# hiroharu-kato/neural_renderer

Hardware: AMD Instinct MI355X
Metric: rasterize fwd+bwd Mpixels/sec @256x256 batch=64 (higher is better)
Workload: dtype f32

## Files before the change

neural_renderer_amd/csrc/nr_backward_pixel_map.hip:

```cpp
#include "nr_device.h"
#include "nr_band_lines.h"
#include "nr_k6_tune.h"

#include <atomic>
#include <mutex>
#include <type_traits>

using namespace nr;

namespace {

constexpr int GRP = 10;
constexpr int NGRP = 6;

struct __attribute__((aligned(16))) LineRec {
    int in_rng;
    int out_rng;
    int base;
    int flags;
    float cross, c0, c1, pad;
    float in_c[4];
    float out_c[4];
};

// ... 101 lines not shown
        const int nl = lane_on ? min(max(n_lines - batch0, 0), GRP) : 0;
        int l = -1, ph = 0, d1 = 0, d1_end = -1, base = 0, cur_flags = 0;
        float cross = 0, c0 = 0, c1 = 0, ref_a = 0, ref_r = 0, ref_g = 0, ref_b = 0;
        while (__ballot(l < nl) != 0ull) {
            if (d1 > d1_end && l < nl) {
                if (ph == 0 && (cur_flags & 2)) ph = 1; else { ph = 0; ++l; }
                if (l < nl) {
                    const LineRec *r = &recs[g][l];
                    const int4 h = *reinterpret_cast<const int4 *>(r);
                    const float4 q = *reinterpret_cast<const float4 *>(&r->cross);
                    const float4 col = *reinterpret_cast<const float4 *>(ph == 0 ? r->out_c : r->in_c);
                    const int rng = ph == 0 ? h.x : h.y;
                    d1 = (rng & 0xffff) + sub;
                    d1_end = rng >> 16;
                    base = h.z;
                    cur_flags = h.w;
                    cross = q.x; c0 = q.y; c1 = q.z;
                    ref_a = col.x; ref_r = col.y; ref_g = col.z; ref_b = col.w;
                }
            }
            if (l < nl && d1 <= d1_end) {
                const int idx = base + d1 * sd1;
                bool skip = (ph == 0) && (fi_map[idx] != fn);
                float diff = 0.0f;
                if (!skip) {
                    if (ALPHA) diff += (alpha_map[idx] - ref_a) * g_alpha[idx];
                    if (RGB) {
                        const float *pp = rgb_map + 3 * (size_t)idx;
                        const float *gg = g_rgb + 3 * (size_t)idx;
                        diff += (pp[0] - ref_r) * gg[0];
                        diff += (pp[1] - ref_g) * gg[1];
                        diff += (pp[2] - ref_b) * gg[2];
                    }
                }
                if (!skip && !(diff <= 0.0f)) {
                    const float t = (float)d1 - cross;
                    if (cur_flags & 4) {
                        const float ct = c0 * t;
                        float dist = (float)(s_pow2 ? (double)ct * two_over_s : (double)ct * 2.0 / s_d);
                        dist = (0.0f < dist) ? (float)((double)dist + eps) : (float)((double)dist - eps);
                        G0 -= (double)(diff / dist);
                    }
                    if (cur_flags & 8) {
                        const float ct = c1 * t;
                        float dist = (float)(s_pow2 ? (double)ct * two_over_s : (double)ct * 2.0 / s_d);
                        dist = (0.0f < dist) ? (float)((double)dist + eps) : (float)((double)dist - eps);
                        G1 -= (double)(diff / dist);
                    }
                }
                d1 += GRP;
            }
        }
        __syncthreads();
    }

#pragma unroll
    for (int o = 8; o > 0; o >>= 1) {
        const double t0 = __shfl_down(G0, o, WAVE), t1 = __shfl_down(G1, o, WAVE);
        if (sub + o < GRP) { G0 += t0; G1 += t1; }
    }
    const int partner = (2 * ((edge + 2) % 3) + axis) * GRP;
    const double G1p = __shfl(G1, partner, WAVE);
    if (lane_on && sub == 0) {
        out[3 * edge + (1 - axis)] = (float)(G0 + G1p);
        if (axis == 0) out[3 * edge + 2] = 0.0f;
    }
}


constexpr int BAND_WIN = 256;
constexpr int FSEG = 15;
enum { K6_FAST = 0, K6_EXACT_POW2 = 1, K6_EXACT = 2 };

__global__ __launch_bounds__(256) void k_mark_visible(const int32_t *__restrict__ fi_map,
                                                      unsigned char *__restrict__ flags, int F, int SS, size_t P)
{
    const size_t i = (size_t)blockIdx.x * blockDim.x + threadIdx.x;
    if (i >= P) return;
    const int fi = fi_map[i];
    if (fi >= 0) flags[(i / SS) * F + fi] = 1;
}

__device__ __forceinline__ void emit_visible(int b, int fn, int pos, int F, int S, const float *__restrict__ faces,
                                             int *__restrict__ vis_list, unsigned *__restrict__ rng,
                                             double *__restrict__ scratch, int *band_count, int n_bands, int W,
                                             int *line_diff = nullptr)
{
    vis_list[(size_t)b * F + pos] = fn;
    const float *f = faces + ((size_t)b * F + fn) * 9;
    const float fs = (float)S;
    float px[3], py[3];
#pragma unroll
    for (int k = 0; k < 3; k++) { px[k] = to_pixel(f[3 * k], fs); py[k] = to_pixel(f[3 * k + 1], fs); }
    unsigned *r0 = rng + (((size_t)b * 2 + 0) * F + pos) * 3, *r1 = rng + (((size_t)b * 2 + 1) * F + pos) * 3;
#pragma unroll
    for (int e = 0; e < 3; e++) {
        const unsigned ra = edge_range(px[e], px[(e + 1) % 3], S), rb = edge_range(py[e], py[(e + 1) % 3], S);
        r0[e] = ra;
        r1[e] = rb;
#pragma unroll
        for (int axis = 0; axis < 2; axis++) {
            const unsigned r = axis ? rb : ra;
            const int lo = (int)(r & 0xffffu), hi = (int)(r >> 16);
            if (line_diff) {
                if (lo <= hi) {
                    atomicAdd(line_diff + axis * (S + 1) + lo, 1);
                    atomicAdd(line_diff + axis * (S + 1) + hi + 1, -1);
                }
                continue;
            }
            for (int band = lo / W; band * W <= hi; ++band)
                atomicAdd(band_count + axis * n_bands + band, min(hi, band * W + W - 1) - max(lo, band * W) + 1);
        }
    }
    double2 *z = reinterpret_cast<double2 *>(scratch + ((size_t)b * F + pos) * 6);
    z[0] = z[1] = z[2] = make_double2(0.0, 0.0);
}

__device__ __forceinline__ void zero_face(float *__restrict__ o)
{
#pragma unroll
    for (int k = 0; k < 9; k++) o[k] = 0.0f;
}

constexpr int VIS_CHUNK = 1024;
constexpr int SMALL_CHUNKS = 16;

__global__ __launch_bounds__(VIS_CHUNK) void k_compact_par(const unsigned char *__restrict__ flags,
                                                           int *__restrict__ vis_list, int *__restrict__ vis_count,
                                                           int *__restrict__ slot_of, int F, int n_chunks,
                                                           const float *__restrict__ faces, unsigned *__restrict__ rng,
                                                           double *__restrict__ scratch, int S,
                                                           int *__restrict__ chunk_band, int n_bands, int W,
                                                           int *__restrict__ band_cursor, float *__restrict__ zero_faces,
                                                           int zero_listed, int use_diff)
{
    extern __shared__ int s_band[];
    __shared__ int s_wcnt[VIS_CHUNK / 64];
    __shared__ int s_part[VIS_CHUNK / 64];
    const int b = blockIdx.y, chunk = blockIdx.x, tid = threadIdx.x, lane = tid & 63, wave = tid >> 6;
    for (int i = tid; i < 2 * n_bands; i += VIS_CHUNK) s_band[i] = 0;
    int *s_diff = use_diff ? s_band + 2 * n_bands : nullptr;
    if (use_diff)
        for (int i = tid; i < 2 * (S + 1); i += VIS_CHUNK) s_diff[i] = 0;
    int part = 0;
    for (int c = 0; c < chunk; ++c) part += __popcll(__ballot(flags[(size_t)b * F + c * VIS_CHUNK + tid] != 0));
    const int fn = chunk * VIS_CHUNK + tid;
    const bool v = fn < F && flags[(size_t)b * F + fn] != 0;
    const unsigned long long m = __ballot(v);
    if (lane == 0) { s_part[wave] = part; s_wcnt[wave] = __popcll(m); }
    __syncthreads();
    int off = 0, own = 0;
    for (int w = 0; w < VIS_CHUNK / 64; ++w) {
        off += s_part[w];
        if (w < wave) off += s_wcnt[w];
        own += s_wcnt[w];
    }
    if (fn < F) {
        const int before = off + __popcll(m & ((1ull << lane) - 1ull));
        slot_of[(size_t)b * F + fn] = v ? before : -1;
        if (v) emit_visible(b, fn, before, F, S, faces, vis_list, rng, scratch, s_band, n_bands, W, s_diff);
        if (zero_faces && (!v || zero_listed)) zero_face(zero_faces + ((size_t)b * F + fn) * 9);
    }
    __syncthreads();
    if (use_diff) {
        const int n2 = 2 * (S + 1), per = (n2 + VIS_CHUNK - 1) / VIS_CHUNK, i0 = tid * per, i1 = min(n2, i0 + per);
        int local = 0;
        for (int i = i0; i < i1; ++i) local += s_diff[i];
        int inc = local;
#pragma unroll
        for (int o = 1; o < 64; o <<= 1) {
            const int t = __shfl_up(inc, o, WAVE);
            if (lane >= o) inc += t;
        }
        __syncthreads();
        if (lane == 63) s_wcnt[wave] = inc;
        __syncthreads();
        int run = inc - local;
        for (int w = 0; w < wave; ++w) run += s_wcnt[w];
        for (int i = i0; i < i1; ++i) {
            run += s_diff[i];
            s_diff[i] = run;
        }
        __syncthreads();
        for (int i = tid; i < 2 * n_bands; i += VIS_CHUNK) {
            const int axis = i >= n_bands, band = i - axis * n_bands;
            int c = 0;
            for (int l = band * W; l < min(S, band * W + W); ++l) c += s_diff[axis * (S + 1) + l];
            s_band[i] = c;
        }
        __syncthreads();
    }
    int *row = chunk_band + ((size_t)b * n_chunks + chunk) * 2 * n_bands;
    for (int i = tid; i < 2 * n_bands; i += VIS_CHUNK) row[i] = s_band[i];
    if (chunk == 0)
        for (int i = tid; i < 2 * n_bands; i += VIS_CHUNK) band_cursor[(size_t)b * 2 * n_bands + i] = 0;
    if (chunk == n_chunks - 1 && tid == 0) {
        int base = 0;
        for (int w = 0; w < VIS_CHUNK / 64; ++w) base += s_part[w];
        vis_count[b] = base + own;
    }
}

__global__ __launch_bounds__(VIS_CHUNK) void k_list_visible(const unsigned char *__restrict__ flags,
                                                            int *__restrict__ vis_list, int *__restrict__ vis_count, int F,
                                                            int n_chunks)
{
    __shared__ int s_wcnt[VIS_CHUNK / 64];
    __shared__ int s_part[VIS_CHUNK / 64];
    const int b = blockIdx.y, chunk = blockIdx.x, tid = threadIdx.x, lane = tid & 63, wave = tid >> 6;
    int part = 0;
    for (int c = 0; c < chunk; ++c) part += __popcll(__ballot(flags[(size_t)b * F + c * VIS_CHUNK + tid] != 0));
    const int fn = chunk * VIS_CHUNK + tid;
    const bool v = fn < F && flags[(size_t)b * F + fn] != 0;
    const unsigned long long m = __ballot(v);
    if (lane == 0) { s_part[wave] = part; s_wcnt[wave] = __popcll(m); }
    __syncthreads();
    int off = 0, own = 0;
    for (int w = 0; w < VIS_CHUNK / 64; ++w) {
        off += s_part[w];
        if (w < wave) off += s_wcnt[w];
        own += s_wcnt[w];
    }
    if (v) vis_list[(size_t)b * F + off + __popcll(m & ((1ull << lane) - 1ull))] = fn;
    if (chunk == n_chunks - 1 && tid == 0) {
        int base = 0;
        for (int w = 0; w < VIS_CHUNK / 64; ++w) base += s_part[w];
        vis_count[b] = base + own;
    }
}

__global__ __launch_bounds__(VIS_CHUNK) void k_count_visible(const unsigned char *__restrict__ flags,
                                                             int *__restrict__ chunk_count, int F, int n_chunks,
                                                             int *__restrict__ band_lines, int n_bands)
{
    __shared__ int s_wcnt[VIS_CHUNK / 64];
    const int b = blockIdx.y, chunk = blockIdx.x, tid = threadIdx.x, lane = tid & 63, wave = tid >> 6;
    for (int i = chunk * VIS_CHUNK + tid; i < 2 * n_bands; i += n_chunks * VIS_CHUNK) band_lines[(size_t)b * 2 * n_bands + i] = 0;
    const int fn = chunk * VIS_CHUNK + tid;
    const bool v = fn < F && flags[(size_t)b * F + fn] != 0;
    const unsigned long long m = __ballot(v);
    if (lane == 0) s_wcnt[wave] = __popcll(m);
    __syncthreads();
    if (tid == 0) {
        int tot = 0;
        for (int w = 0; w < VIS_CHUNK / 64; ++w) tot += s_wcnt[w];
        chunk_count[(size_t)b * n_chunks + chunk] = tot;
    }
}

__global__ __launch_bounds__(VIS_CHUNK) void k_compact_visible(const unsigned char *__restrict__ flags,
                                                               const int *__restrict__ chunk_count,
                                                               int *__restrict__ vis_list, int *__restrict__ vis_count,
                                                               int *__restrict__ slot_of, int F, int n_chunks,
                                                               const float *__restrict__ faces,
                                                               unsigned *__restrict__ rng, double *__restrict__ scratch,
                                                               int S, int *__restrict__ band_lines, int n_bands, int W,
                                                               int lds_counters, float *__restrict__ zero_faces,
                                                               int zero_listed)
{
    extern __shared__ int s_band[];
    __shared__ int s_wcnt[VIS_CHUNK / 64];
    __shared__ int s_part[VIS_CHUNK / 64];
    const int b = blockIdx.y, chunk = blockIdx.x, tid = threadIdx.x, lane = tid & 63, wave = tid >> 6;
    if (lds_counters)
        for (int i = tid; i < 2 * n_bands; i += VIS_CHUNK) s_band[i] = 0;
    int part = 0;
    for (int c = tid; c < chunk; c += VIS_CHUNK) part += chunk_count[(size_t)b * n_chunks + c];
#pragma unroll
    for (int o = 32; o > 0; o >>= 1) part += __shfl_xor(part, o, WAVE);
    const int fn = chunk * VIS_CHUNK + tid;
    const bool v = fn < F && flags[(size_t)b * F + fn] != 0;
    const unsigned long long m = __ballot(v);
    if (lane == 0) { s_part[wave] = part; s_wcnt[wave] = __popcll(m); }
    __syncthreads();
    int off = 0, own = 0;
    for (int w = 0; w < VIS_CHUNK / 64; ++w) {
        off += s_part[w];
        if (w < wave) off += s_wcnt[w];
        own += s_wcnt[w];
    }
    if (fn < F) {
        const int before = off + __popcll(m & ((1ull << lane) - 1ull));
        slot_of[(size_t)b * F + fn] = v ? before : -1;
        if (zero_faces && (!v || zero_listed)) zero_face(zero_faces + ((size_t)b * F + fn) * 9);
        if (v)
            emit_visible(b, fn, before, F, S, faces, vis_list, rng, scratch,
                         lds_counters ? s_band : band_lines + (size_t)b * 2 * n_bands, n_bands, W);
    }
    if (lds_counters) {
        __syncthreads();
        for (int i = tid; i < 2 * n_bands; i += VIS_CHUNK) {
            const int c = s_band[i];
            if (c) atomicAdd(band_lines + (size_t)b * 2 * n_bands + i, c);
        }
    }
    if (chunk == n_chunks - 1 && tid == 0) {
        int base = 0;
        for (int w = 0; w < VIS_CHUNK / 64; ++w) base += s_part[w];
        vis_count[b] = base + own;
    }
}

template <int NT>
__device__ __forceinline__ int block_excl_scan(int v, int *s_tmp, int *total)
{
    const int tid = threadIdx.x, lane = tid & 63, wave = tid >> 6;
    int inc = v;
#pragma unroll
    for (int o = 1; o < 64; o <<= 1) {
        const int t = __shfl_up(inc, o, WAVE);
        if (lane >= o) inc += t;
    }
    if (lane == 63) s_tmp[wave] = inc;
    __syncthreads();
    int woff = 0, tot = 0;
    for (int w = 0; w < NT / 64; ++w) {
        const int c = s_tmp[w];
        if (w < wave) woff += c;
        tot += c;
    }
    __syncthreads();
    *total = tot;
    return woff + inc - v;
}

__device__ __forceinline__ double signed_eps(float dist, unsigned eps_hi, unsigned eps_lo)
{
    return __hiloint2double((int)((0.0f < dist) ? eps_hi : (eps_hi ^ 0x80000000u)), (int)eps_lo);
}

__global__ __launch_bounds__(256) void k_line_setup(LineSetupArgs a) { line_setup_body(a, (int)blockIdx.x, (int)blockIdx.y); }

__device__ __forceinline__ void band_prefix(const int *cnt, int n2, int *__restrict__ start_out, int *__restrict__ cursor_out,
                                            int *__restrict__ ok_out, size_t cap)
{
    if (threadIdx.x >= 64) return;
    const int lane = threadIdx.x, per = (n2 + 63) / 64;
    int local = 0;
    for (int i = lane * per; i < min(n2, (lane + 1) * per); ++i) local += cnt[i];
    int inc = local;
#pragma unroll
    for (int o = 1; o < 64; o <<= 1) {
        const int t = __shfl_up(inc, o, WAVE);
        if (lane >= o) inc += t;
    }
    int run = inc - local;
    for (int i = lane * per; i < min(n2, (lane + 1) * per); ++i) {
        start_out[i] = run;
        cursor_out[i] = 0;
        run += cnt[i];
    }
    const int total = __shfl(inc, 63, WAVE);
    if (lane == 0) *ok_out = ((size_t)total <= cap) ? 1 : 0;
}

__global__ __launch_bounds__(256) void k_band_scan(const int *__restrict__ band_lines, int *__restrict__ band_start,
                                                   int *__restrict__ band_cursor, int *__restrict__ lines_ok, int n_bands,
                                                   size_t cap, int force_scan)
{
    const size_t o = (size_t)blockIdx.x * 2 * n_bands;
    band_prefix(band_lines + o, 2 * n_bands, band_start + o, band_cursor + o, lines_ok + blockIdx.x, force_scan ? 0 : cap);
}

__global__ __launch_bounds__(256) void k_band_total(const int *__restrict__ chunk_band, int n_sum, int *__restrict__ band_lines,
                                                    int *__restrict__ band_start, int *__restrict__ lines_ok, int n_bands)
{
    const int b = blockIdx.x, n2 = 2 * n_bands;
    const int *rows = chunk_band + (size_t)b * n_sum * n2;
    for (int i = threadIdx.x; i < n2; i += blockDim.x) {
        int t = 0;
        for (int c = 0; c < n_sum; ++c) t += rows[(size_t)c * n2 + i];
        band_lines[(size_t)b * n2 + i] = t;
        band_start[(size_t)b * n2 + i] = 0;
    }
    if (threadIdx.x == 0) lines_ok[b] = 0;
}

struct FastPx {
    int *fi;
    float *g;
    float *c;
    float *bg;
    unsigned *cov;
    int CW;
    int *span;
};

template <bool RGB, bool ALPHA, int NT>
__device__ __forceinline__ void fast_stage(const FastPx &px, const int32_t *__restrict__ fi_map,
                                           const float *__restrict__ rgb_map, const float *__restrict__ alpha_map,
                                           const float *__restrict__ g_rgb, const float *__restrict__ g_alpha, size_t img,
                                           int axis, int band_lo, int nld, int S, int SP)
{
    const int tid = threadIdx.x;
    auto put = [&](int ld, int d1, int fi, float al, float ga, float r, float g, float bl, float gr, float gg, float gb) {
        const int l = ld * SP + d1;
        px.fi[l] = fi;
        if (RGB) {
            *reinterpret_cast<float4 *>(px.g + 4 * (size_t)l) = make_float4(ga, gr, gg, gb);
            *reinterpret_cast<float4 *>(px.c + 4 * (size_t)l) = make_float4(al, r, g, bl);
            if (px.bg && fi < 0) *reinterpret_cast<float4 *>(px.bg) = make_float4(al, r, g, bl);
        } else {
            px.g[l] = ga;
            px.c[l] = al;
            if (px.bg && fi < 0) px.bg[0] = al;
        }
        if (px.cov && fi >= 0) atomicOr(px.cov + ld * px.CW + (d1 >> 5), 1u << (d1 & 31));
    };
    auto put_quad = [&](size_t g, int ld0, int d10, int ld_step, int d1_step) {
        const int4 vf = *reinterpret_cast<const int4 *>(fi_map + g);
        float4 va = make_float4(0, 0, 0, 0), vg = va;
        if (ALPHA) {
            va = *reinterpret_cast<const float4 *>(alpha_map + g);
            vg = *reinterpret_cast<const float4 *>(g_alpha + g);
// ... 1106 lines not shown
                            used(gD);
                            __builtin_amdgcn_sched_barrier(0);
                            gp += 4 * (SEG * NC * 4);
                            pp += 4 * SEG;
                            pf += (float)(4 * SEG);
                        }
                        if (const int rem = steps2 - s) {
                            if (rem == 3) load(2, gC, pC);
                            visit(gA, pA, pf, a0, a1);
                            used(gA);
                            if (rem >= 2) {
                                visit(gB, pB, pf + (float)SEG, b0, b1);
                                used(gB);
                            }
                            if (rem == 3) {
                                visit(gC, pC, pf + (float)(2 * SEG), a0, a1);
                                used(gC);
                            }
                        }
                    }
                    A0 = __builtin_amdgcn_mfma_f64_4x4x4f64((double)a0, 1.0, 0.0, 0, 0, 0);
                    A1 = __builtin_amdgcn_mfma_f64_4x4x4f64((double)a1, 1.0, 0.0, 0, 0, 0);
                    A0 = __builtin_amdgcn_mfma_f64_4x4x4f64((double)b0, 1.0, A0, 0, 0, 0);
                    A1 = __builtin_amdgcn_mfma_f64_4x4x4f64((double)b1, 1.0, A1, 0, 0, 0);
                    A0 = __builtin_amdgcn_mfma_f64_4x4x4f64(A0, 1.0, 0.0, 0, 0, 0);
                    A1 = __builtin_amdgcn_mfma_f64_4x4x4f64(A1, 1.0, 0.0, 0, 0, 0);
                }
                if (act && lane == (row << 2)) acc[src] = make_double2(A0, A1);
            }
            wave_lds_handover();
            if (lane < nw) {
                double2 a = make_double2(0.0, 0.0);
                if (has_b && ((pos >> 2) & (team - 1)) == member) a = acc[lane];
                a.x += (double)f0;
                a.y += (double)f1;
                const bool tneg = !dpos;
                const bool neg0 = EXACT || (((__float_as_uint(qq.y) >> 31) != 0) != tneg);
                const bool neg1 = EXACT || (((__float_as_uint(qq.z) >> 31) != 0) != tneg);
                const double t0 = (flags & 2) ? in0 + (neg0 ? a.x : -a.x) : 0.0;
                const double t1 = (flags & 4) ? in1 + (neg1 ? a.y : -a.y) : 0.0;
                const int tgt = hh.w, lpos = tgt & 0x0fffffff;
                double *dst = scratch + ((size_t)b * F + lpos) * 6 + (1 - axis);
                if (t0 != 0.0) atomicAdd(dst + 2 * ((tgt >> 28) & 3), t0);
                if (t1 != 0.0) atomicAdd(dst + 2 * ((tgt >> 30) & 3), t1);
            }
            wave_lds_handover();
        }
    }
}

__global__ __launch_bounds__(256) void k_bpm_finalize(const double *__restrict__ scratch, const int *__restrict__ slot_of,
                                                      float *__restrict__ grad_faces, int F, int n_faces_total, int add)
{
    const int i = blockIdx.x * blockDim.x + threadIdx.x;
    if (i >= n_faces_total) return;
    const int pos = slot_of[i];
    float *o = grad_faces + (size_t)i * 9;
    if (add) {
        if (pos < 0) return;
        const double *src = scratch + ((size_t)(i / F) * F + pos) * 6;
#pragma unroll
        for (int v = 0; v < 3; v++) {
            o[3 * v + 0] = (float)src[2 * v + 0] + o[3 * v + 0];
            o[3 * v + 1] = (float)src[2 * v + 1] + o[3 * v + 1];
        }
        return;
    }
    double a[6] = {0.0, 0.0, 0.0, 0.0, 0.0, 0.0};
    if (pos >= 0) {
        const double *src = scratch + ((size_t)(i / F) * F + pos) * 6;
#pragma unroll
        for (int k = 0; k < 6; k++) a[k] = src[k];
    }
#pragma unroll
    for (int v = 0; v < 3; v++) {
        o[3 * v + 0] = (float)a[2 * v + 0];
        o[3 * v + 1] = (float)a[2 * v + 1];
        o[3 * v + 2] = 0.0f;
    }
}


struct BpmLayout {
    size_t flags_off, scratch_off, count_off, chunk_off, cband_off, list_off, rng_off, slot_off, band_off, start_off, cursor_off, ok_off,
        lines_off, total, cap;
    int n_chunks;
};

size_t line_capacity(int F, int S)
{
    const size_t want = (size_t)8 * F + (size_t)32 * S + (size_t)(1.2 * (double)S * sqrt((double)F));
    return (want + 2047 - 1088) / 2048 * 2048 + 1088;
}

BpmLayout bpm_layout(int B, int F, int S)
{
    BpmLayout L;
    const size_t n = (size_t)B * F;
    L.flags_off = 0;
    L.scratch_off = align_up(n, 256);
    L.count_off = align_up(L.scratch_off + n * 6 * sizeof(double), 256);
    L.n_chunks = (F + VIS_CHUNK - 1) / VIS_CHUNK;
    L.chunk_off = L.count_off + align_up((size_t)B * sizeof(int), 256);
    L.cband_off = L.chunk_off + align_up((size_t)B * L.n_chunks * sizeof(int), 256);
    L.list_off = L.cband_off + (L.n_chunks <= SMALL_CHUNKS ? align_up((size_t)B * L.n_chunks * 2 * S * sizeof(int), 256) : 0);
    L.rng_off = L.list_off + align_up(n * sizeof(int), 256);
    L.slot_off = L.rng_off + align_up(n * 6 * sizeof(unsigned), 256);
    const size_t per_band = align_up((size_t)B * 2 * S * sizeof(int), 256);
    L.band_off = L.slot_off + align_up(n * sizeof(int), 256);
    L.start_off = L.band_off + per_band;
    L.cursor_off = L.start_off + per_band;
    L.ok_off = L.cursor_off + per_band;
    L.lines_off = L.ok_off + align_up((size_t)B * sizeof(int), 256);
    L.cap = line_capacity(F, S);
    L.total = L.lines_off + (size_t)B * L.cap * sizeof(BandLine);
    return L;
}

struct ListsLayout {
    size_t count_off, list_off, total;
};
ListsLayout lists_layout(int B, int F)
{
    ListsLayout L;
    L.count_off = 0;
    L.list_off = align_up((size_t)B * sizeof(int), 256);
    L.total = L.list_off + (size_t)B * F * sizeof(int);
    return L;
}

struct BandShape {
    int threads;
    int w_max;
    size_t budget;
};
BandShape band_shape(int S)
{
    if (S <= k6::SMALL_RASTER_MAX) return {256, 2, (size_t)40 * 1024};
    if (S > k6::WIDE_BUDGET_FROM && S <= k6::WIDE_BUDGET_TO) return {512, k6::WMAX, (size_t)80 * 1024};
    return {512, k6::WMAX, k6::LDS_BUDGET};
}

int fast_band_config(int S, bool rgb, const BandShape &shape, int w_max, size_t *lds_bytes, int *win, int *qcap)
{
    const size_t per_px = rgb ? 36 : 12, SP = (size_t)S + 4, dsz = S > 63 * FSEG ? 4 : 2;
    const size_t segs_per_line = (size_t)S / (S <= 320 ? 32 : 48) + 3;
    const size_t NT = (size_t)shape.threads, LDS_BUDGET = shape.budget;
    const int win_max = BAND_WIN < shape.threads ? BAND_WIN : shape.threads;
    auto lines_bytes = [&](int ww) { return (sizeof(BandLine) + 16) * (size_t)ww; };
    for (int W = w_max; W >= 1; W >>= 1) {
        const size_t px = (size_t)W * SP * per_px + (size_t)W * (((SP + 31) / 32 + 3) / 4 * 4) * 4 + 16  + 32  + 64  +
                          8 * 16 ;
        const size_t lim = (W == 1 && px + lines_bytes(32) + NT * dsz > LDS_BUDGET) ? 160 * 1024 : LDS_BUDGET;
        if (px + lines_bytes(32) + NT * dsz > lim) continue;
        const size_t rest = lim - px;
        int w = (int)(rest / (48 + segs_per_line * dsz));
        w = max(32, min(win_max, w / 32 * 32));
        while (w > 32 && lines_bytes(w) + NT * dsz > rest) w -= 32;
        if (W > 1 && w < 96) continue;
        size_t q = (rest - lines_bytes(w)) / dsz / NT * NT;
        q = q > 16384 ? 16384 : q;
        *win = w;
        *qcap = (int)q;
        *lds_bytes = px + lines_bytes(w) + q * dsz;
        return W;
    }
    return 0;
}

struct LdsLimit {
    std::atomic<size_t> granted[32];
    std::mutex mtx;
    LdsLimit() { for (auto &g : granted) g.store(48 * 1024); }
    int ensure(const void *kern, size_t lds)
    {
        int dev = 0;
        if (hipGetDevice(&dev) != hipSuccess || dev < 0 || dev >= 32) dev = 31;
        if (lds <= granted[dev].load(std::memory_order_acquire) && dev != 31) return 0;
        std::lock_guard<std::mutex> lock(mtx);
        const size_t have = granted[dev].load(std::memory_order_relaxed);
        if (lds <= have && dev != 31) return 0;
        const size_t want = lds > have ? lds : have;
        const hipError_t e = hipFuncSetAttribute(kern, hipFuncAttributeMaxDynamicSharedMemorySize, (int)want);
        if (e != 0) return e;
        granted[dev].store(want, std::memory_order_release);
        return 0;
    }
};

enum K6Kernel { K6_KERNEL_FAST = 0, K6_KERNEL_ROW = 1, K6_KERNEL_GLOBAL = 2 };
// ... 146 lines not shown
    BandKernelTimer &t = g_band_timer;
    if (enable && !t.start) {
        if (hipEventCreate(&t.start) != hipSuccess || hipEventCreate(&t.stop) != hipSuccess) {
            t.start = t.stop = nullptr;
            return launch_status();
        }
    }
    t.on = enable != 0 && t.start != nullptr;
    t.recorded = false;
    return 0;
}

NR_API float nr_profile_band_kernel_ms(void)
{
    BandKernelTimer &t = g_band_timer;
    float ms = -1.0f;
    if (!t.recorded || hipEventSynchronize(t.stop) != hipSuccess || hipEventElapsedTime(&ms, t.start, t.stop) != hipSuccess) {
        (void)hipGetLastError();
        return -1.0f;
    }
    return ms;
}
NR_API int nr_profile_band_kernel_which(void) { return g_band_timer.recorded ? g_band_timer.which : -1; }
NR_API int nr_profile_k6_choice(int32_t B, int32_t F, int32_t S, int32_t return_rgb, int32_t return_alpha, double eps, int32_t flags)
{
    (void)return_alpha;
    return plan_k6(B, F, S, return_rgb != 0, eps, flags).kernel == K6_KERNEL_ROW ? 1 : 0;
}
#define NR_BAND_TIMER_START(st, kernel) if (g_band_timer.on) { g_band_timer.which = (kernel); g_band_timer.recorded = hipEventRecord(g_band_timer.start, st) == hipSuccess; }
#define NR_BAND_TIMER_STOP(st) if (g_band_timer.on && g_band_timer.recorded) g_band_timer.recorded = hipEventRecord(g_band_timer.stop, st) == hipSuccess
#else
#define NR_BAND_TIMER_START(st, kernel) ((void)0)
#define NR_BAND_TIMER_STOP(st) ((void)0)
#endif

int nr::run_backward_pixel_map(const float *faces, const int32_t *face_index_map, const float *rgb_map,
                               const float *alpha_map, const float *grad_rgb_map, const float *grad_alpha_map,
                               float *grad_faces, int B, int F, int S, double eps, int return_rgb, int return_alpha,
                               int flags, const unsigned char *visible_faces, void *workspace, size_t workspace_bytes,
                               hipStream_t st, const int **vis_list_out, const int **vis_count_out,
                               const double **defer_scratch, const int **defer_slot_of, void *zero_ptr, size_t zero_bytes,
                               int *zeroed, const SetupHook *hook)
{
    if (zeroed) *zeroed = 0;
    if (vis_list_out) *vis_list_out = nullptr;
    if (vis_count_out) *vis_count_out = nullptr;
    if (defer_scratch) *defer_scratch = nullptr;
    if (defer_slot_of) *defer_slot_of = nullptr;
    if (!faces || !face_index_map || !grad_faces) return NR_E_NULL;
    if (!return_rgb && !return_alpha) return NR_E_MODE;
    if (return_rgb && (!rgb_map || !grad_rgb_map)) return NR_E_NULL;
    if (return_alpha && (!alpha_map || !grad_alpha_map)) return NR_E_NULL;
    if (int e = check_sizes(B, F, S)) return e;
    if ((size_t)B * S * S > 0x7fffffffull / 3) return NR_E_SIZE;
    const int n = B * F;
    const bool rgb = return_rgb != 0, alpha = return_alpha != 0;
    const bool exact = (flags & NR_FLAG_EXACT_GRADIENT) != 0;
    const K6Plan plan = plan_k6(B, F, S, rgb, eps, flags);
    if (plan.kernel == K6_KERNEL_GLOBAL) {
        const dim3 grid((unsigned)n), block(WAVE);
        if (rgb && alpha)
            hipLaunchKernelGGL((k_bpm_global<true, true>), grid, block, 0, st, faces, face_index_map, rgb_map,
                               alpha_map, grad_rgb_map, grad_alpha_map, grad_faces, F, S, eps);
        else if (rgb)
            hipLaunchKernelGGL((k_bpm_global<true, false>), grid, block, 0, st, faces, face_index_map, rgb_map,
                               alpha_map, grad_rgb_map, grad_alpha_map, grad_faces, F, S, eps);
        else
            hipLaunchKernelGGL((k_bpm_global<false, true>), grid, block, 0, st, faces, face_index_map, rgb_map,
                               alpha_map, grad_rgb_map, grad_alpha_map, grad_faces, F, S, eps);
        return launch_status();
    }

    const BpmLayout L = bpm_layout(B, F, S);
    if (!workspace || workspace_bytes < L.total) return NR_E_WORKSPACE;
    const bool defer = defer_scratch && defer_slot_of;
    unsigned char *ws = (unsigned char *)workspace;
    int *band_lines = (int *)(ws + L.band_off);
    const int W = plan.W, n_bands = plan.n_bands;
    double *scratch = (double *)(ws + L.scratch_off);
    int *vis_count = (int *)(ws + L.count_off);
    int *vis_list = (int *)(ws + L.list_off);
    int *slot_of = (int *)(ws + L.slot_off);
    unsigned *rng = (unsigned *)(ws + L.rng_off);
    if (vis_list_out) *vis_list_out = vis_list;
    if (vis_count_out) *vis_count_out = vis_count;
    const unsigned char *vflags = visible_faces;
    if (!vflags) {
        unsigned char *f = ws + L.flags_off;
        const int he = fill_bytes(f, 0, (size_t)n, st);
        if (he != 0) return he;
        const size_t P = (size_t)B * S * S;
        hipLaunchKernelGGL(k_mark_visible, dim3((unsigned)((P + 255) / 256)), dim3(256), 0, st, face_index_map, f, F,
                           S * S, P);
        vflags = f;
    }
    int *band_start = (int *)(ws + L.start_off), *band_cursor = (int *)(ws + L.cursor_off), *lines_ok = (int *)(ws + L.ok_off);
    BandLine *line_buf = (BandLine *)(ws + L.lines_off);
    const bool use_records = plan.use_records;
    const float k2s = exact ? 1.0f : 2.0f / (float)S;
    const size_t cap = use_records ? L.cap : 0;
    int n_sum = 0;
    if (L.n_chunks <= SMALL_CHUNKS && n_bands <= 4096) {
        int *chunk_band = (int *)(ws + L.cband_off);
        n_sum = L.n_chunks;
        const int use_diff = (size_t)(2 * n_bands + 2 * (S + 1)) * sizeof(int) <= 40960 ? 1 : 0;
        hipLaunchKernelGGL(k_compact_par, dim3((unsigned)L.n_chunks, (unsigned)B), dim3(VIS_CHUNK),
                           (size_t)(2 * n_bands + (use_diff ? 2 * (S + 1) : 0)) * sizeof(int), st, vflags, vis_list, vis_count,
                           slot_of, F, L.n_chunks, faces, rng, scratch, S, chunk_band, n_bands, W, band_cursor,
                           defer ? grad_faces : (float *)nullptr, hook ? 1 : 0, use_diff);
        if (!use_records)
            hipLaunchKernelGGL(k_band_total, dim3((unsigned)B), dim3(256), 0, st, chunk_band, n_sum, band_lines, band_start,
                               lines_ok, n_bands);
    } else {
        int *chunk_count = (int *)(ws + L.chunk_off);
        hipLaunchKernelGGL(k_count_visible, dim3((unsigned)L.n_chunks, (unsigned)B), dim3(VIS_CHUNK), 0, st, vflags,
                           chunk_count, F, L.n_chunks, band_lines, n_bands);
        const int lds_counters = n_bands <= 4096;
        hipLaunchKernelGGL(k_compact_visible, dim3((unsigned)L.n_chunks, (unsigned)B), dim3(VIS_CHUNK),
                           lds_counters ? (size_t)2 * n_bands * sizeof(int) : 0, st, vflags, chunk_count, vis_list, vis_count,
                           slot_of, F, L.n_chunks, faces, rng, scratch, S, band_lines, n_bands, W, lds_counters,
                           defer ? grad_faces : (float *)nullptr, hook ? 1 : 0);
        hipLaunchKernelGGL(k_band_scan, dim3((unsigned)B), dim3(256), 0, st, band_lines, band_start, band_cursor, lines_ok,
                           n_bands, cap, 0);
    }
    {
        const LineSetupArgs la = {faces, face_index_map, vis_list, vis_count, rng, (const int *)(ws + L.cband_off), n_sum, band_lines,
                                  band_start, band_cursor, lines_ok, line_buf, L.cap, F, S, W, n_bands, k2s,
                                  (unsigned)((F + LS_FACES - 1) / LS_FACES), (unsigned)B, (size_t)6 * n_bands * sizeof(int)};
        if (hook) {
            if (int rc = hook->launch(hook->ctx, use_records ? &la : nullptr, vis_list, vis_count, slot_of, st)) return rc;
        } else if (use_records) {
            if (int rc = run_line_setup(la, st)) return rc;
        }
    }
    const bool zero_ok = !hook && zero_ptr && zero_bytes > 0 && zero_bytes % 16 == 0 && ((size_t)zero_ptr & 15) == 0 &&
                         zero_bytes <= plan.fill_max;
    void *const fill_ptr = zero_ok ? zero_ptr : nullptr;
    const size_t fill_len = zero_ok ? zero_bytes : 0;
    auto band_fast = [&](auto overflow_only, void *zp, size_t zb) {
        return with_k6_types(rgb, alpha, plan.mode, [&](auto r, auto a, auto m) {
            return launch_fast<decltype(r)::value, decltype(a)::value, decltype(m)::value, decltype(overflow_only)::value>(
                plan, faces, face_index_map, rgb_map, alpha_map, grad_rgb_map, grad_alpha_map, vis_list, vis_count, rng, scratch,
                band_lines, band_start, lines_ok, line_buf, L.cap, B, F, S, eps, k2s, st, zp, zb);
        });
    };
    auto band_row = [&]() {
        return with_k6_types(rgb, alpha, plan.mode, [&](auto r, auto a, auto m) {
            return launch_row<decltype(r)::value, decltype(a)::value, decltype(m)::value>(
                plan, face_index_map, rgb_map, alpha_map, grad_rgb_map, grad_alpha_map, scratch, band_lines, band_start, lines_ok,
                line_buf, L.cap, B, F, S, eps, st, fill_ptr, fill_len);
        });
    };
    NR_BAND_TIMER_START(st, plan.kernel);
    int rc = plan.kernel == K6_KERNEL_ROW ? band_row() : band_fast(std::false_type(), fill_ptr, fill_len);
    NR_BAND_TIMER_STOP(st);
    if (rc == 0 && plan.overflow_pass) rc = band_fast(std::true_type(), nullptr, 0);
    if (rc) return rc;
    if (zero_ok && zeroed) *zeroed = 1;
    if (defer) {
        *defer_scratch = scratch;
        *defer_slot_of = slot_of;
        return launch_status();
    }
    hipLaunchKernelGGL(k_bpm_finalize, dim3((unsigned)((n + 255) / 256)), dim3(256), 0, st, scratch, slot_of, grad_faces,
                       F, n, 0);
    return launch_status();
}

void nr::run_bpm_finalize(const double *scratch, const int *slot_of, float *grad_faces, int B, int F, hipStream_t st, bool add)
{
    const int n = B * F;
    hipLaunchKernelGGL(k_bpm_finalize, dim3((unsigned)((n + 255) / 256)), dim3(256), 0, st, scratch, slot_of, grad_faces,
                       F, n, add ? 1 : 0);
}

int nr::run_line_setup(const LineSetupArgs &a, hipStream_t st)
{
    static LdsLimit ls_limit;
    if (int rc = ls_limit.ensure((const void *)k_line_setup, a.lds_bytes)) return rc;
    hipLaunchKernelGGL(k_line_setup, dim3(a.grid_x, a.grid_y), dim3(256), a.lds_bytes, st, a);
    return launch_status();
}

NR_API int nr_backward_pixel_map(const float *faces, const int32_t *face_index_map, const float *rgb_map,
                                 const float *alpha_map, const float *grad_rgb_map, const float *grad_alpha_map,
                                 float *grad_faces, int32_t B, int32_t F, int32_t S, double eps, int32_t return_rgb,
                                 int32_t return_alpha, int32_t flags, const uint8_t *visible_faces, void *workspace,
                                 size_t workspace_bytes, void *stream)
{
    return run_backward_pixel_map(faces, face_index_map, rgb_map, alpha_map, grad_rgb_map, grad_alpha_map, grad_faces, B,
                                  F, S, eps, return_rgb, return_alpha, flags, visible_faces, workspace, workspace_bytes,
                                  (hipStream_t)stream, nullptr, nullptr);
}

namespace {
struct GatherCall {
    const float *faces, *faces_z_ref, *weight_map, *depth_map, *grad_rgb_map, *grad_depth_map;
    const int32_t *face_index_map;
    float *grad_textures, *grad_faces;
    int B, F, S, ts, flags;
    double eps;
    const FaceLight *lit;
    bool called;
    int depth_done;
};

int launch_setup_and_gather(void *ctx, const LineSetupArgs *ls, const int *vis_list, const int *vis_count, const int *slot_of,
                            hipStream_t st)
{
// ... 106 lines not shown
```

neural_renderer_amd/csrc/nr_band_lines.h:

```cpp
#pragma once
#include "nr_device.h"

namespace nr {

struct __attribute__((aligned(16))) BandLine {
    int in_rng;
    int out_rng;
    int geo;
    int tgt;
    float cross, c0, c1;
    int fn;
};

struct LineSetupArgs {
    const float *faces;
    const int32_t *fi_map;
    const int *vis_list, *vis_count;
    const unsigned *rng;
    const int *chunk_band;
    int n_sum;
    int *band_lines, *band_start, *band_cursor, *lines_ok;
    BandLine *line_buf;
    size_t cap;
    int F, S, W, n_bands;
    float k2s;
    unsigned grid_x, grid_y;
    size_t lds_bytes;
};

int run_line_setup(const LineSetupArgs &a, hipStream_t st);

struct SetupHook {
    int (*launch)(void *ctx, const LineSetupArgs *ls, const int *vis_list, const int *vis_count, const int *slot_of,
                  hipStream_t st);
    void *ctx;
};

namespace {


constexpr unsigned RNG_EMPTY = 1u;

__device__ __forceinline__ unsigned edge_range(float p0x, float p1x, int S)
{
    const int d0_from = (int)fmax((double)ceilf(fminf(p0x, p1x)), 0.0);
    const int d0_to = (int)fmin((double)fmaxf(p0x, p1x), S - 1.0);
    return (p0x != p1x && d0_to >= d0_from) ? (unsigned)d0_from | ((unsigned)d0_to << 16) : RNG_EMPTY;
}


struct LineHead {
    float p0x, p0y, p1x, p1y, p2x, p2y, d0f, d1_cross;
    int direction, d1_in, d1_out;
    bool live;
};

__device__ __forceinline__ LineHead fast_line_head(const float *__restrict__ fv, int e, int axis, int d0, int S)
{
    const float fs = (float)S;
    const int i0 = e, i1 = (e + 1) % 3, i2 = (e + 2) % 3;
    float fp[6];
#pragma unroll
    for (int k = 0; k < 3; k++) { fp[k] = to_pixel(fv[3 * k], fs); fp[3 + k] = to_pixel(fv[3 * k + 1], fs); }
    const int ox = axis ? 3 : 0, oy = axis ? 0 : 3;
    LineHead h;
    h.p0x = fp[ox + i0]; h.p0y = fp[oy + i0]; h.p1x = fp[ox + i1]; h.p1y = fp[oy + i1];
    h.p2x = fp[ox + i2]; h.p2y = fp[oy + i2];
    if (axis == 0) h.direction = (h.p0x < h.p1x) ? -1 : 1; else h.direction = (h.p0x < h.p1x) ? 1 : -1;
    h.d0f = (float)d0;
    h.d1_cross = (h.p1y - h.p0y) / (h.p1x - h.p0x) * (h.d0f - h.p0x) + h.p0y;
    h.d1_in = (0 < h.direction) ? (int)floorf(h.d1_cross) : (int)ceilf(h.d1_cross);
    h.d1_out = h.d1_in + h.direction;
    h.live = !(h.d1_in < 0 || S <= h.d1_in) && !(h.d1_out < 0 || S <= h.d1_out);
    return h;
}

__device__ __forceinline__ BandLine fast_line_finish(const LineHead &h, int ld, int S, int rfn, int tgt, int owner, float k2s)
{
    const float p0x = h.p0x, p0y = h.p0y, p1x = h.p1x, p1y = h.p1y, p2x = h.p2x, p2y = h.p2y, d0f = h.d0f;
    const int direction = h.direction, d1_in = h.d1_in, d1_out = h.d1_out;
    BandLine r;
    r.in_rng = 1; r.out_rng = 1; r.geo = 0; r.tgt = tgt;
    r.cross = r.c0 = r.c1 = 0.0f;
    r.fn = rfn;
    if (h.live) {
        int flags = (0 < direction) ? 8 : 0;
        if (p1x != d0f) flags |= 2;
        if (p0x != d0f) flags |= 4;
        r.c0 = (p1x - p0x) / (p1x - d0f) * k2s;
        r.c1 = (p1x - p0x) / (d0f - p0x) * k2s;
        if (owner == rfn) {
            const int lim = (0 < direction) ? S - 1 : 0;
            const int o_from = max(min(d1_out, lim), 0), o_to = min(max(d1_out, lim), S - 1);
            r.out_rng = o_from | (o_to << 16);
            flags |= 1;
        }
        float d0_cross2;
        if ((d0f - p0x) * (d0f - p2x) < 0)
            d0_cross2 = (p2y - p0y) / (p2x - p0x) * (d0f - p0x) + p0y;
        else
            d0_cross2 = (p1y - p2y) / (p1x - p2x) * (d0f - p2x) + p2y;
        const int lim2 = (0 < direction) ? (int)ceilf(d0_cross2) : (int)floorf(d0_cross2);
        const int i_from = max(min(d1_in, lim2), 0), i_to = min(max(d1_in, lim2), S - 1);
        r.in_rng = i_from | (i_to << 16);
        r.geo = d1_in | (ld << 16) | (flags << 24);
        r.cross = h.d1_cross;
    }
    return r;
}

template <typename OwnerOf>
__device__ __forceinline__ BandLine make_fast_line(const float *__restrict__ fv, int e, int axis, int d0, int ld, int S,
                                                   int rfn, int tgt, OwnerOf owner_of, float k2s)
{
    const LineHead h = fast_line_head(fv, e, axis, d0, S);
    return fast_line_finish(h, ld, S, rfn, tgt, h.live ? owner_of(h.d1_in) : -1, k2s);
}

constexpr int LS_UNROLL = 4;
constexpr int LS_FACES = 32;

__device__ __forceinline__ int band_sum_prefix(const int *__restrict__ rows, int n_sum, int n2, int *tot, int *start,
                                               int *s_tmp)
{
    const int tid = threadIdx.x, lane = tid & 63, wave = tid >> 6;
    for (int i = tid; i < n2; i += 256) {
        int t = 0;
        for (int c = 0; c < n_sum; ++c) t += rows[(size_t)c * n2 + i];
        tot[i] = t;
    }
    __syncthreads();
    const int per = (n2 + 255) / 256, i0 = tid * per, i1 = min(n2, i0 + per);
    int local = 0;
    for (int i = i0; i < i1; ++i) local += tot[i];
    int inc = local;
#pragma unroll
    for (int o = 1; o < 64; o <<= 1) {
        const int t = __shfl_up(inc, o, WAVE);
        if (lane >= o) inc += t;
    }
    if (lane == 63) s_tmp[wave] = inc;
    __syncthreads();
    int run = inc - local;
    for (int w = 0; w < wave; ++w) run += s_tmp[w];
    for (int i = i0; i < i1; ++i) {
        start[i] = run;
        run += tot[i];
    }
    const int total = s_tmp[0] + s_tmp[1] + s_tmp[2] + s_tmp[3];
    __syncthreads();
    return total;
}

__device__ __forceinline__ void line_setup_body(const LineSetupArgs &a, const int bx, const int by)
{
    const float *__restrict__ faces = a.faces;
    const int32_t *__restrict__ fi_map = a.fi_map;
    const int *__restrict__ vis_list = a.vis_list, *__restrict__ vis_count = a.vis_count;
    const unsigned *__restrict__ rng = a.rng;
    const int *__restrict__ chunk_band = a.chunk_band;
    const int n_sum = a.n_sum;
    int *__restrict__ band_lines = a.band_lines, *__restrict__ band_start = a.band_start, *__restrict__ band_cursor = a.band_cursor,
        *__restrict__ lines_ok = a.lines_ok;
    BandLine *__restrict__ line_buf = a.line_buf;
    const size_t cap = a.cap;
    const int F = a.F, S = a.S, W = a.W, n_bands = a.n_bands;
    const float k2s = a.k2s;
    extern __shared__ int s_cnt[];
    int *s_base = s_cnt + 2 * n_bands;
    int *s_start = s_base + 2 * n_bands;
    __shared__ int s_tmp[4];
    __shared__ unsigned s_rng[6 * LS_FACES];
    __shared__ int s_lp[6 * LS_FACES + 1];
    __shared__ int s_fn[LS_FACES];
    __shared__ float s_face[9 * LS_FACES];
    const int b = by, tid = threadIdx.x;
    const bool first = bx == 0;
    const int n_vis = vis_count[b];
    const int n_wg = (n_vis + LS_FACES - 1) / LS_FACES;
    const int pos0 = bx, pstep = n_wg;
    const int n_pos = bx < n_wg ? (n_vis - pos0 + pstep - 1) / pstep : 0;
    if (n_pos == 0 && !first) return;
    unsigned r_own = RNG_EMPTY;
    int fn_own = 0;
    if (tid < 6 * n_pos) {
        const int p = tid / 6, ae = tid - 6 * p, axis = ae / 3, e = ae - 3 * axis;
        r_own = rng[(((size_t)b * 2 + axis) * F + pos0 + p * pstep) * 3 + e];
    }
    if (tid < n_pos) fn_own = vis_list[(size_t)b * F + pos0 + tid * pstep];
    int ok;
    if (n_sum > 0) {
        const int total = band_sum_prefix(chunk_band + (size_t)b * n_sum * 2 * n_bands, n_sum, 2 * n_bands, s_cnt, s_start, s_tmp);
        ok = (size_t)total <= cap ? 1 : 0;
        if (first) {
            for (int i = tid; i < 2 * n_bands; i += 256) {
                band_lines[(size_t)b * 2 * n_bands + i] = s_cnt[i];
                band_start[(size_t)b * 2 * n_bands + i] = s_start[i];
            }
            if (tid == 0) lines_ok[b] = ok;
        }
    } else {
        ok = lines_ok[b];
        for (int i = tid; i < 2 * n_bands; i += 256) s_start[i] = band_start[(size_t)b * 2 * n_bands + i];
    }
    if (n_pos == 0 || !ok) return;
    __syncthreads();
    for (int i = tid; i < 2 * n_bands; i += 256) s_cnt[i] = 0;
    if (tid < 6 * LS_FACES) s_rng[tid] = r_own;
    if (tid < LS_FACES) s_fn[tid] = fn_own;
    __syncthreads();
    float fv_a = 0.0f, fv_b = 0.0f;
    {
        const int p = tid / 9, k = tid - 9 * p;
        if (p < n_pos) fv_a = faces[((size_t)b * F + s_fn[p]) * 9 + k];
        const int t2 = tid + 256, p2 = t2 / 9, k2 = t2 - 9 * p2;
        if (t2 < 9 * LS_FACES && p2 < n_pos) fv_b = faces[((size_t)b * F + s_fn[p2]) * 9 + k2];
    }
    {
        int lines = 0;
        if (tid < 6 * n_pos) {
            const int p = tid / 6, ae = tid - 6 * p, axis = ae / 3;
            const unsigned pr = s_rng[tid];
            const int lo = (int)(pr & 0xffffu), hi = (int)(pr >> 16);
            for (int band = lo / W; band * W <= hi; ++band)
                atomicAdd(s_cnt + axis * n_bands + band, min(hi, band * W + W - 1) - max(lo, band * W) + 1);
            lines = hi >= lo ? hi - lo + 1 : 0;
        }
        const int lane = tid & 63, wave = tid >> 6;
        int inc = lines;
#pragma unroll
        for (int o = 1; o < 64; o <<= 1) {
            const int t = __shfl_up(inc, o, WAVE);
            if (lane >= o) inc += t;
        }
        if (lane == 63) s_tmp[wave] = inc;
        __syncthreads();
        int before = 0;
        for (int w = 0; w < wave; ++w) before += s_tmp[w];
        if (tid < 6 * LS_FACES) s_lp[tid] = before + inc - lines;
        if (tid == 6 * LS_FACES - 1) s_lp[6 * LS_FACES] = before + inc;
    }
    __syncthreads();
    for (int i = tid; i < 2 * n_bands; i += 256) {
        const int c = s_cnt[i];
        s_base[i] = c > 0 ? s_start[i] + atomicAdd(band_cursor + (size_t)b * 2 * n_bands + i, c) : 0;
        s_cnt[i] = 0;
    }
    s_face[tid] = fv_a;
    if (tid + 256 < 9 * LS_FACES) s_face[tid + 256] = fv_b;
    __syncthreads();
    const size_t img = (size_t)b * S * S;
    BandLine *buf_b = line_buf + (size_t)b * cap;
    const int n_items = 6 * n_pos, n_lines = s_lp[n_items];
    for (int base = 0; base < n_lines; base += LS_UNROLL * 256) {
        LineHead h[LS_UNROLL];
        int item[LS_UNROLL], d0v[LS_UNROLL], own[LS_UNROLL];
#pragma unroll
        for (int u = 0; u < LS_UNROLL; u++) {
            const int l = base + u * 256 + tid;
            item[u] = -1;
            own[u] = -1;
            if (l < n_lines) {
                int lo = 0, hi = n_items;
                while (hi - lo > 1) {
                    const int mid = (lo + hi) >> 1;
                    if (s_lp[mid] <= l) lo = mid; else hi = mid;
                }
                item[u] = lo;
                const int p = lo / 6, ae = lo - 6 * p, axis = ae / 3, e = ae - 3 * axis;
                const int d0 = (int)(s_rng[lo] & 0xffffu) + (l - s_lp[lo]);
                d0v[u] = d0;
                float fv[9];
#pragma unroll
                for (int k = 0; k < 9; k++) fv[k] = s_face[9 * p + k];
                h[u] = fast_line_head(fv, e, axis, d0, S);
                if (h[u].live) own[u] = fi_map[axis ? img + (size_t)d0 * S + h[u].d1_in : img + (size_t)h[u].d1_in * S + d0];
            }
        }
#pragma unroll
        for (int u = 0; u < LS_UNROLL; u++) {
            if (item[u] < 0) continue;
            const int p = item[u] / 6, ae = item[u] - 6 * p, axis = ae / 3, e = ae - 3 * axis;
            const int band = d0v[u] / W, ld = d0v[u] - band * W;
            const int tgt = (pos0 + p * pstep) | (e << 28) | (((e + 1) % 3) << 30);
            const int bi = axis * n_bands + band;
            buf_b[s_base[bi] + atomicAdd(s_cnt + bi, 1)] = fast_line_finish(h[u], ld, S, s_fn[p], tgt, own[u], k2s);
        }
    }
}

}
}
```

Baseline: 14070.

## Precompute pixel-space vertices in compaction and overlap line heads with band reservation

The compaction kernels now write each visible face's six pixel-space vertex coordinates into a new workspace array. Line setup reads these instead of gathering nine raw face floats through the vis list and converting them again, which shrinks shared memory and drops a dependent gather. The first batch of line heads, including their fi_map loads, is now computed before the band cursor atomics, so the global atomic latency overlaps with head work. The unroll is reduced from 4 to 2 and the line-setup grid index is remapped so batches are interleaved across block order. The cost is an extra workspace buffer with its write and read traffic.

After: 14260, median of 6. 1.01x the previous value.

```diff
diff --git a/neural_renderer_amd/csrc/nr_backward_pixel_map.hip b/neural_renderer_amd/csrc/nr_backward_pixel_map.hip
--- a/neural_renderer_amd/csrc/nr_backward_pixel_map.hip
+++ b/neural_renderer_amd/csrc/nr_backward_pixel_map.hip
@@ -207,7 +207,7 @@
 }
 
 __device__ __forceinline__ void emit_visible(int b, int fn, int pos, int F, int S, const float *__restrict__ faces,
-                                             int *__restrict__ vis_list, unsigned *__restrict__ rng,
+                                             int *__restrict__ vis_list, unsigned *__restrict__ rng, float *__restrict__ pix,
                                              double *__restrict__ scratch, int *band_count, int n_bands, int W,
                                              int *line_diff = nullptr)
 {
@@ -217,6 +217,10 @@
     float px[3], py[3];
 #pragma unroll
     for (int k = 0; k < 3; k++) { px[k] = to_pixel(f[3 * k], fs); py[k] = to_pixel(f[3 * k + 1], fs); }
+    float2 *pv = reinterpret_cast<float2 *>(pix + ((size_t)b * F + pos) * 6);
+    pv[0] = make_float2(px[0], px[1]);
+    pv[1] = make_float2(px[2], py[0]);
+    pv[2] = make_float2(py[1], py[2]);
     unsigned *r0 = rng + (((size_t)b * 2 + 0) * F + pos) * 3, *r1 = rng + (((size_t)b * 2 + 1) * F + pos) * 3;
 #pragma unroll
     for (int e = 0; e < 3; e++) {
@@ -255,7 +259,7 @@
                                                            int *__restrict__ vis_list, int *__restrict__ vis_count,
                                                            int *__restrict__ slot_of, int F, int n_chunks,
                                                            const float *__restrict__ faces, unsigned *__restrict__ rng,
-                                                           double *__restrict__ scratch, int S,
+                                                           float *__restrict__ pix, double *__restrict__ scratch, int S,
                                                            int *__restrict__ chunk_band, int n_bands, int W,
                                                            int *__restrict__ band_cursor, float *__restrict__ zero_faces,
                                                            int zero_listed, int use_diff)
@@ -284,7 +288,7 @@
     if (fn < F) {
         const int before = off + __popcll(m & ((1ull << lane) - 1ull));
         slot_of[(size_t)b * F + fn] = v ? before : -1;
-        if (v) emit_visible(b, fn, before, F, S, faces, vis_list, rng, scratch, s_band, n_bands, W, s_diff);
+        if (v) emit_visible(b, fn, before, F, S, faces, vis_list, rng, pix, scratch, s_band, n_bands, W, s_diff);
         if (zero_faces && (!v || zero_listed)) zero_face(zero_faces + ((size_t)b * F + fn) * 9);
     }
     __syncthreads();
@@ -379,8 +383,8 @@
                                                                int *__restrict__ vis_list, int *__restrict__ vis_count,
                                                                int *__restrict__ slot_of, int F, int n_chunks,
                                                                const float *__restrict__ faces,
-                                                               unsigned *__restrict__ rng, double *__restrict__ scratch,
-                                                               int S, int *__restrict__ band_lines, int n_bands, int W,
+                                                               unsigned *__restrict__ rng, float *__restrict__ pix,
+                                                               double *__restrict__ scratch, int S, int *__restrict__ band_lines, int n_bands, int W,
                                                                int lds_counters, float *__restrict__ zero_faces,
                                                                int zero_listed)
 {
@@ -410,7 +414,7 @@
         slot_of[(size_t)b * F + fn] = v ? before : -1;
         if (zero_faces && (!v || zero_listed)) zero_face(zero_faces + ((size_t)b * F + fn) * 9);
         if (v)
-            emit_visible(b, fn, before, F, S, faces, vis_list, rng, scratch,
+            emit_visible(b, fn, before, F, S, faces, vis_list, rng, pix, scratch,
                          lds_counters ? s_band : band_lines + (size_t)b * 2 * n_bands, n_bands, W);
     }
     if (lds_counters) {
@@ -455,7 +459,11 @@
     return __hiloint2double((int)((0.0f < dist) ? eps_hi : (eps_hi ^ 0x80000000u)), (int)eps_lo);
 }
 
-__global__ __launch_bounds__(256) void k_line_setup(LineSetupArgs a) { line_setup_body(a, (int)blockIdx.x, (int)blockIdx.y); }
+__global__ __launch_bounds__(256) void k_line_setup(LineSetupArgs a)
+{
+    const unsigned lin = blockIdx.y * gridDim.x + blockIdx.x, nb = gridDim.y;
+    line_setup_body(a, (int)(lin / nb), (int)(lin % nb));
+}
 
 __device__ __forceinline__ void band_prefix(const int *cnt, int n2, int *__restrict__ start_out, int *__restrict__ cursor_out,
                                             int *__restrict__ ok_out, size_t cap)
@@ -1728,8 +1736,8 @@
 
 
 struct BpmLayout {
-    size_t flags_off, scratch_off, count_off, chunk_off, cband_off, list_off, rng_off, slot_off, band_off, start_off, cursor_off, ok_off,
-        lines_off, total, cap;
+    size_t flags_off, scratch_off, count_off, chunk_off, cband_off, list_off, rng_off, pix_off, slot_off, band_off, start_off,
+        cursor_off, ok_off, lines_off, total, cap;
     int n_chunks;
 };
 
@@ -1751,7 +1759,8 @@
     L.cband_off = L.chunk_off + align_up((size_t)B * L.n_chunks * sizeof(int), 256);
     L.list_off = L.cband_off + (L.n_chunks <= SMALL_CHUNKS ? align_up((size_t)B * L.n_chunks * 2 * S * sizeof(int), 256) : 0);
     L.rng_off = L.list_off + align_up(n * sizeof(int), 256);
-    L.slot_off = L.rng_off + align_up(n * 6 * sizeof(unsigned), 256);
+    L.pix_off = L.rng_off + align_up(n * 6 * sizeof(unsigned), 256);
+    L.slot_off = L.pix_off + align_up(n * 6 * sizeof(float), 256);
     const size_t per_band = align_up((size_t)B * 2 * S * sizeof(int), 256);
     L.band_off = L.slot_off + align_up(n * sizeof(int), 256);
     L.start_off = L.band_off + per_band;
@@ -2064,6 +2073,7 @@
     int *vis_list = (int *)(ws + L.list_off);
     int *slot_of = (int *)(ws + L.slot_off);
     unsigned *rng = (unsigned *)(ws + L.rng_off);
+    float *pix = (float *)(ws + L.pix_off);
     if (vis_list_out) *vis_list_out = vis_list;
     if (vis_count_out) *vis_count_out = vis_count;
     const unsigned char *vflags = visible_faces;
@@ -2088,7 +2098,7 @@
         const int use_diff = (size_t)(2 * n_bands + 2 * (S + 1)) * sizeof(int) <= 40960 ? 1 : 0;
         hipLaunchKernelGGL(k_compact_par, dim3((unsigned)L.n_chunks, (unsigned)B), dim3(VIS_CHUNK),
                            (size_t)(2 * n_bands + (use_diff ? 2 * (S + 1) : 0)) * sizeof(int), st, vflags, vis_list, vis_count,
-                           slot_of, F, L.n_chunks, faces, rng, scratch, S, chunk_band, n_bands, W, band_cursor,
+                           slot_of, F, L.n_chunks, faces, rng, pix, scratch, S, chunk_band, n_bands, W, band_cursor,
                            defer ? grad_faces : (float *)nullptr, hook ? 1 : 0, use_diff);
         if (!use_records)
             hipLaunchKernelGGL(k_band_total, dim3((unsigned)B), dim3(256), 0, st, chunk_band, n_sum, band_lines, band_start,
@@ -2100,13 +2110,13 @@
         const int lds_counters = n_bands <= 4096;
         hipLaunchKernelGGL(k_compact_visible, dim3((unsigned)L.n_chunks, (unsigned)B), dim3(VIS_CHUNK),
                            lds_counters ? (size_t)2 * n_bands * sizeof(int) : 0, st, vflags, chunk_count, vis_list, vis_count,
-                           slot_of, F, L.n_chunks, faces, rng, scratch, S, band_lines, n_bands, W, lds_counters,
+                           slot_of, F, L.n_chunks, faces, rng, pix, scratch, S, band_lines, n_bands, W, lds_counters,
                            defer ? grad_faces : (float *)nullptr, hook ? 1 : 0);
         hipLaunchKernelGGL(k_band_scan, dim3((unsigned)B), dim3(256), 0, st, band_lines, band_start, band_cursor, lines_ok,
                            n_bands, cap, 0);
     }
     {
-        const LineSetupArgs la = {faces, face_index_map, vis_list, vis_count, rng, (const int *)(ws + L.cband_off), n_sum, band_lines,
+        const LineSetupArgs la = {pix, face_index_map, vis_list, vis_count, rng, (const int *)(ws + L.cband_off), n_sum, band_lines,
                                   band_start, band_cursor, lines_ok, line_buf, L.cap, F, S, W, n_bands, k2s,
                                   (unsigned)((F + LS_FACES - 1) / LS_FACES), (unsigned)B, (size_t)6 * n_bands * sizeof(int)};
         if (hook) {
diff --git a/neural_renderer_amd/csrc/nr_band_lines.h b/neural_renderer_amd/csrc/nr_band_lines.h
--- a/neural_renderer_amd/csrc/nr_band_lines.h
+++ b/neural_renderer_amd/csrc/nr_band_lines.h
@@ -13,7 +13,7 @@
 };
 
 struct LineSetupArgs {
-    const float *faces;
+    const float *pix;
     const int32_t *fi_map;
     const int *vis_list, *vis_count;
     const unsigned *rng;
@@ -55,13 +55,9 @@
     bool live;
 };
 
-__device__ __forceinline__ LineHead fast_line_head(const float *__restrict__ fv, int e, int axis, int d0, int S)
-{
-    const float fs = (float)S;
+__device__ __forceinline__ LineHead line_head(const float *fp, int e, int axis, int d0, int S)
+{
     const int i0 = e, i1 = (e + 1) % 3, i2 = (e + 2) % 3;
-    float fp[6];
-#pragma unroll
-    for (int k = 0; k < 3; k++) { fp[k] = to_pixel(fv[3 * k], fs); fp[3 + k] = to_pixel(fv[3 * k + 1], fs); }
     const int ox = axis ? 3 : 0, oy = axis ? 0 : 3;
     LineHead h;
     h.p0x = fp[ox + i0]; h.p0y = fp[oy + i0]; h.p1x = fp[ox + i1]; h.p1y = fp[oy + i1];
@@ -73,6 +69,15 @@
     h.d1_out = h.d1_in + h.direction;
     h.live = !(h.d1_in < 0 || S <= h.d1_in) && !(h.d1_out < 0 || S <= h.d1_out);
     return h;
+}
+
+__device__ __forceinline__ LineHead fast_line_head(const float *__restrict__ fv, int e, int axis, int d0, int S)
+{
+    const float fs = (float)S;
+    float fp[6];
+#pragma unroll
+    for (int k = 0; k < 3; k++) { fp[k] = to_pixel(fv[3 * k], fs); fp[3 + k] = to_pixel(fv[3 * k + 1], fs); }
+    return line_head(fp, e, axis, d0, S);
 }
 
 __device__ __forceinline__ BandLine fast_line_finish(const LineHead &h, int ld, int S, int rfn, int tgt, int owner, float k2s)
@@ -117,7 +122,7 @@
     return fast_line_finish(h, ld, S, rfn, tgt, h.live ? owner_of(h.d1_in) : -1, k2s);
 }
 
-constexpr int LS_UNROLL = 4;
+constexpr int LS_UNROLL = 2;
 constexpr int LS_FACES = 32;
 
 __device__ __forceinline__ int band_sum_prefix(const int *__restrict__ rows, int n_sum, int n2, int *tot, int *start,
@@ -154,7 +159,7 @@
 
 __device__ __forceinline__ void line_setup_body(const LineSetupArgs &a, const int bx, const int by)
 {
-    const float *__restrict__ faces = a.faces;
+    const float *__restrict__ pix = a.pix;
     const int32_t *__restrict__ fi_map = a.fi_map;
     const int *__restrict__ vis_list = a.vis_list, *__restrict__ vis_count = a.vis_count;
     const unsigned *__restrict__ rng = a.rng;
@@ -173,7 +178,7 @@
     __shared__ unsigned s_rng[6 * LS_FACES];
     __shared__ int s_lp[6 * LS_FACES + 1];
     __shared__ int s_fn[LS_FACES];
-    __shared__ float s_face[9 * LS_FACES];
+    __shared__ float s_pix[6 * LS_FACES];
     const int b = by, tid = threadIdx.x;
     const bool first = bx == 0;
     const int n_vis = vis_count[b];
@@ -182,10 +187,13 @@
     const int n_pos = bx < n_wg ? (n_vis - pos0 + pstep - 1) / pstep : 0;
     if (n_pos == 0 && !first) return;
     unsigned r_own = RNG_EMPTY;
+    float p_own = 0.0f;
     int fn_own = 0;
     if (tid < 6 * n_pos) {
         const int p = tid / 6, ae = tid - 6 * p, axis = ae / 3, e = ae - 3 * axis;
-        r_own = rng[(((size_t)b * 2 + axis) * F + pos0 + p * pstep) * 3 + e];
+        const size_t pos = (size_t)pos0 + (size_t)p * pstep;
+        r_own = rng[(((size_t)b * 2 + axis) * F + pos) * 3 + e];
+        p_own = pix[((size_t)b * F + pos) * 6 + ae];
     }
     if (tid < n_pos) fn_own = vis_list[(size_t)b * F + pos0 + tid * pstep];
     int ok;
@@ -206,16 +214,9 @@
     if (n_pos == 0 || !ok) return;
     __syncthreads();
     for (int i = tid; i < 2 * n_bands; i += 256) s_cnt[i] = 0;
-    if (tid < 6 * LS_FACES) s_rng[tid] = r_own;
+    if (tid < 6 * LS_FACES) { s_rng[tid] = r_own; s_pix[tid] = p_own; }
     if (tid < LS_FACES) s_fn[tid] = fn_own;
     __syncthreads();
-    float fv_a = 0.0f, fv_b = 0.0f;
-    {
-        const int p = tid / 9, k = tid - 9 * p;
-        if (p < n_pos) fv_a = faces[((size_t)b * F + s_fn[p]) * 9 + k];
-        const int t2 = tid + 256, p2 = t2 / 9, k2 = t2 - 9 * p2;
-        if (t2 < 9 * LS_FACES && p2 < n_pos) fv_b = faces[((size_t)b * F + s_fn[p2]) * 9 + k2];
-    }
     {
         int lines = 0;
         if (tid < 6 * n_pos) {
@@ -241,20 +242,12 @@
         if (tid == 6 * LS_FACES - 1) s_lp[6 * LS_FACES] = before + inc;
     }
     __syncthreads();
-    for (int i = tid; i < 2 * n_bands; i += 256) {
-        const int c = s_cnt[i];
-        s_base[i] = c > 0 ? s_start[i] + atomicAdd(band_cursor + (size_t)b * 2 * n_bands + i, c) : 0;
-        s_cnt[i] = 0;
-    }
-    s_face[tid] = fv_a;
-    if (tid + 256 < 9 * LS_FACES) s_face[tid + 256] = fv_b;
-    __syncthreads();
     const size_t img = (size_t)b * S * S;
     BandLine *buf_b = line_buf + (size_t)b * cap;
     const int n_items = 6 * n_pos, n_lines = s_lp[n_items];
-    for (int base = 0; base < n_lines; base += LS_UNROLL * 256) {
-        LineHead h[LS_UNROLL];
-        int item[LS_UNROLL], d0v[LS_UNROLL], own[LS_UNROLL];
+    LineHead h[LS_UNROLL];
+    int item[LS_UNROLL], d0v[LS_UNROLL], own[LS_UNROLL];
+    auto heads = [&](int base) {
 #pragma unroll
         for (int u = 0; u < LS_UNROLL; u++) {
             const int l = base + u * 256 + tid;
@@ -270,13 +263,15 @@
                 const int p = lo / 6, ae = lo - 6 * p, axis = ae / 3, e = ae - 3 * axis;
                 const int d0 = (int)(s_rng[lo] & 0xffffu) + (l - s_lp[lo]);
                 d0v[u] = d0;
-                float fv[9];
-#pragma unroll
-                for (int k = 0; k < 9; k++) fv[k] = s_face[9 * p + k];
-                h[u] = fast_line_head(fv, e, axis, d0, S);
+                float fp[6];
+#pragma unroll
+                for (int k = 0; k < 6; k++) fp[k] = s_pix[6 * p + k];
+                h[u] = line_head(fp, e, axis, d0, S);
                 if (h[u].live) own[u] = fi_map[axis ? img + (size_t)d0 * S + h[u].d1_in : img + (size_t)h[u].d1_in * S + d0];
             }
         }
+    };
+    auto finish = [&]() {
 #pragma unroll
         for (int u = 0; u < LS_UNROLL; u++) {
             if (item[u] < 0) continue;
@@ -286,8 +281,20 @@
             const int bi = axis * n_bands + band;
             buf_b[s_base[bi] + atomicAdd(s_cnt + bi, 1)] = fast_line_finish(h[u], ld, S, s_fn[p], tgt, own[u], k2s);
         }
-    }
-}
-
-}
-}
+    };
+    heads(0);
+    for (int i = tid; i < 2 * n_bands; i += 256) {
+        const int c = s_cnt[i];
+        s_base[i] = c > 0 ? s_start[i] + atomicAdd(band_cursor + (size_t)b * 2 * n_bands + i, c) : 0;
+        s_cnt[i] = 0;
+    }
+    __syncthreads();
+    finish();
+    for (int base = LS_UNROLL * 256; base < n_lines; base += LS_UNROLL * 256) {
+        heads(base);
+        finish();
+    }
+}
+
+}
+}
```
